# VatsalPandey0202/PointCloudRegistration

Measured on AMD Instinct MI355X. Metric: TOF/PC pairs/sec (8192 pts), higher is better.
Workload: dtype f32 xyz/features; f64 RANSAC/ICP; 1-term f16 MFMA screen (certified bound), f16x3-split MFMA screen for the rows it leaves, f64 exact re-rank; 1 GPU; C4: batch of augmented TOF/PC pairs (featNN+RANSAC+ICP+Chamfer); pairs_total=256, pairs_per_gpu=256, points=8192, feature_dim=32, streams_per_gpu=1, ransac=d=0.04 mutual n=3 edge0.9 dist0.04 (100000,0.999), icp=d=0.02 (1e-6,1e-6,30), parallelism=pair-sharded x1, inputs=resident in HBM (--full: host_resident is the PCIe-inclusive rate)

## Files before the change

pointcloudregistration_amd/csrc/featnn.hip:

```cpp
#include "featnn_v5.h"
#include "scan.h"
#include <stdlib.h>
#include <algorithm>

namespace pcr {
namespace {

__global__ __launch_bounds__(1024) void corres_build(const int32_t *nn12, const int32_t *nn21,
                                                     const int32_t *n_src, const int32_t *n_tgt,
                                                     int Nmax, int Mmax, int mutual, int ransac_n,
                                                     int *scratch, int32_t *corres,
                                                     int32_t *n_corres) {
    const int p = blockIdx.x;
    const int n = count_of(n_src, p, Nmax);
    const int m = count_of(n_tgt, p, Mmax);
    const int32_t *a12 = nn12 + (size_t)p * Nmax;
    const int32_t *a21 = nn21 + (size_t)p * Mmax;
    int *f = scratch + (size_t)p * (Nmax + 1);
    int32_t *co = corres + (size_t)p * Nmax * 2;
    for (int i = threadIdx.x; i < n; i += 1024) {
        const int j = a12[i];
        f[i] = (mutual && j >= 0 && j < m && a21[j] == i) ? 1 : 0;
    }
    __syncthreads();
// ... 147 lines not shown
static int beside(hipStream_t s, Side side, Main main) {
    static const bool off = [] {
        const char *e = getenv("PCR_FEAT_BESIDE");
        return !(e && e[0] == '1');
    }();
    hipStream_t q = s;
    hipEvent_t ef = nullptr, ej = nullptr;
    int rc = off ? PCR_OK : side_stream(&q, &ef, &ej, 2);
    if (rc != PCR_OK) return rc;
    if (q != s) {
        PCR_HIP_CHECK(hipEventRecord(ef, s));
        PCR_HIP_CHECK(hipStreamWaitEvent(q, ef, 0));
    }
    if ((rc = side(q)) != PCR_OK) return rc;
    if (q != s) PCR_HIP_CHECK(hipEventRecord(ej, q));
    prof_begin(s, kProfFeatRegroup);
    rc = main();
    prof_end(s, kProfFeatRegroup);
    if (rc != PCR_OK) return rc;
    if (q != s) PCR_HIP_CHECK(hipStreamWaitEvent(s, ej, 0));
    return PCR_OK;
}

static bool feat_one_term() {
    const char *e = getenv("PCR_FEAT_ONE");
    return !(e && e[0] == '0');
}


template <bool kIdx>
static int run_pass(const RowArgs5 &r, const RowArgs5 &fb, int S, bool one, bool use9, int slot, int slot_fb,
                    int *llist, int *lcount, hipStream_t s) {
    int rc;
    prof_begin(s, slot);
    if (use9) {
        PCR_HIP_CHECK(hipMemsetAsync(r.bcnt, 0, sizeof(int) * (size_t)r.P * (r.ntc / 2), s));
        if ((rc = launch_row9<kIdx>(r, S, s)) != PCR_OK) return rc;
        prof_end(s, slot);
        RowArgs5 rg = r;
        rg.llist = llist; rg.lcount = lcount;
        return beside(s, [&](hipStream_t q) { return launch_fallback<kIdx>(fb, S, q, slot_fb); },
                      [&] { return launch_regroup9<kIdx>(rg, S, s); });
    }
    if (one) rc = launch_row8<kIdx, true>(r, S, s);
    else if (S <= 2) rc = launch_row8<kIdx, false>(r, S, s);
    else rc = launch_row7<kIdx>(r, S, s);
    if (rc != PCR_OK) return rc;
    prof_end(s, slot);
    return one ? launch_fallback<kIdx>(fb, S, s, slot_fb) : PCR_OK;
}

static RowArgs5 fallback_args(RowArgs5 r, int *list, int *count, int fbdiag, int fsl) {
    r.rlist = r.list; r.rcount = r.count;
    r.list = list; r.count = count;
    r.fbdiag = fbdiag; r.rbmajor = 1; r.csl = fsl;
    return r;
}

static int feature_corres_v5(const float *F, const float *G, int P, int Nmax, int Mmax, int D,
                             const int32_t *n_src, const int32_t *n_tgt, int mutual, int ransac_n,
                             int32_t *nn12, int32_t *corres, int32_t *n_corres, hipStream_t s) {
    V5Buf v;
    int rc = v5_prepare(F, G, P, Nmax, Mmax, D, n_src, n_tgt, s, v);
    if (rc != PCR_OK) return rc;
    const int ntn = v.ntn, ntm = v.ntm;
    const size_t pn = (size_t)P * Nmax, pm = (size_t)P * Mmax;
    const int nst1 = ntm / 2, nst2 = ntn / 2;
    const int cap1 = std::max(64, 4 * cdiv(Nmax, nst1)), cap2 = std::max(64, 4 * cdiv(Mmax, nst2));
    const size_t pb = (size_t)P * std::max(nst1, nst2);
    const size_t pl = (size_t)P * std::max((size_t)nst1 * cap1, (size_t)nst2 * cap2);
    const size_t pr = (size_t)P * std::max(Nmax, Mmax);
    const int fsl = list_slices(P);
    const size_t pt = fsl > 1 ? (size_t)fsl * pr : 0;
    MutArgs ma;
    double *v12;
    float *e12;
    float4 *wq;
    int *nn21x, *zero, *bcnt;
    int32_t *nns;
    uint4 *blist, *rec, *part;
    WsLayout l;
    l.take(v12, pn); l.take(e12, pn);
    l.take(wq, pm);
    l.take(ma.used, pm + P); l.take(ma.pos, pm + P);
    l.take(ma.jlist, pm); l.take(nn21x, pm);
    l.take(ma.flag, pn + P);
    l.take(ma.nj, P); l.take(zero, P);
    l.take(nns, pn);
    l.take(blist, pl);
    l.take(rec, pr); l.take(part, pt);
    l.take(bcnt, pb);
    bool fresh = false;
    PCR_REQUIRE(workspace_bind(kWsFeatMutual, l, kWsSlack + 32, &fresh), PCR_ERR_NOMEM, "feature_corres: %s",
                pcr_last_error());
    const bool one = v.S <= 2 && feat_one_term();
    const bool use9 = one && feat_row9() && std::max(ntm, ntn) / 2 <= kRegroupMaxSteps;
    static thread_local const void *z_ptr = nullptr;
    static thread_local int z_cnt = 0;
    if (fresh || z_ptr != (const void *)zero || z_cnt < P) {
        PCR_HIP_CHECK(hipMemsetAsync(zero, 0, sizeof(int) * (size_t)P, s));
        z_ptr = zero;
        z_cnt = P;
    }
    ma.nn12 = nn12; ma.n_src = n_src; ma.n_tgt = n_tgt; ma.Nmax = Nmax; ma.Mmax = Mmax;
    ma.mutual = mutual; ma.ransac_n = ransac_n; ma.Kt = 16 * v.NX; ma.D = D; ma.ntm = ntm;
    ma.v12 = v12; ma.e12 = e12; ma.wq = wq; ma.fmax = v.fmax;
    ma.nns = v.S <= 2 ? nns : nn12;
    ma.F = F; ma.G = G; ma.mx = v.mx;
    ma.list21 = v.list21; ma.cnt21 = v.cnt21; ma.nn21x = nn21x;
    ma.corres = corres; ma.n_corres = n_corres;
    RowArgs5 r;
    r.Ap = v.Ap; r.Bp = v.Bp; r.rnr = v.fnr; r.cmax = v.gmax; r.n_rows = n_src; r.n_cols = n_tgt;
    r.rlist = nullptr; r.rcount = nullptr; r.P = P; r.Rmax = Nmax; r.Cmax = Mmax; r.ntr = ntn;
    r.ntc = ntm; r.nrb = 0; r.D = D; r.ctbits = 1;
    while ((1 << r.ctbits) < ntm) ++r.ctbits;
    r.nn = nn12; r.v = v12; r.e = e12;
    r.list = one ? v.fbl12 : v.list12; r.count = one ? v.fbc12 : v.cnt12;
    r.wq = nullptr;
    r.Xr = F; r.sc = v.mx; r.role = 0; r.cs = v.sp.cs;
    r.cemax = v.gemax; r.nns = nns; r.fbdiag = 0; r.rbmajor = 0;
    r.rre = v.fre; r.bcnt = bcnt; r.blist = blist; r.bcap = cap1; r.rec = rec;
    r.cct = v.gct; r.rct = v.fct; r.cbias = v.cbias;
    r.csl = 1; r.part = part; r.llist = nullptr; r.lcount = nullptr;
    auto prep_hook = [&](int at) -> int {
        if (!prep_event || prep_at != at) return PCR_OK;
        PCR_HIP_CHECK(hipEventRecord(prep_event, s));
        const int hrc = prep_fn ? prep_fn(prep_ctx) : PCR_OK;
        if (hrc == PCR_OK) prep_fn = nullptr;
        return hrc;
    };
    if ((rc = prep_hook(2)) != PCR_OK) return rc;
    rc = run_pass<true>(r, fallback_args(r, v.list12, v.cnt12, 1, fsl), v.S, one, use9, kProfFeatScreen,
                        kProfFeatScreen1b, v.list12, v.cnt12, s);
    if (rc != PCR_OK) return rc;
    if ((rc = prep_hook(1)) != PCR_OK) return rc;
    RescanArgs5 ra = rescan_args(F, G, n_src, n_tgt, Nmax, Mmax, D);
    ra.list12 = v.list12; ra.list21 = v.list21; ra.cnt12 = v.cnt12; ra.cnt21 = zero;
    ra.nn12 = nn12; ra.nn21 = nn21x;
    ra.v12 = v12; ra.e12 = e12; ra.mx = v.mx; ra.T = v.sp.T;
    hipStream_t rs = s;
    hipEvent_t ev_fork = nullptr, ev_join = nullptr;
    if (mutual && P >= 192) {
        rc = side_stream(&rs, &ev_fork, &ev_join, 1);
        if (rc != PCR_OK) return rc;
        PCR_HIP_CHECK(hipEventRecord(ev_fork, s));
        PCR_HIP_CHECK(hipStreamWaitEvent(rs, ev_fork, 0));
    }
    rc = run_rescan(ra, P, D, rs);
    if (rc != PCR_OK) return rc;
    if (rs != s) PCR_HIP_CHECK(hipEventRecord(ev_join, rs));
    if (mutual) {
        const size_t jsm = sizeof(int) * ((size_t)Mmax + 1);
        static size_t jstatic = [] {
            hipFuncAttributes fa{};
            return hipFuncGetAttributes(&fa, (const void *)featmut_jbuild<true>) == hipSuccess
                       ? fa.sharedSizeBytes : (size_t)1024;
        }();
        if (jsm + jstatic <= 64 * 1024) {
            PCR_HIP_CHECK(hipFuncSetAttribute((const void *)featmut_jbuild<true>,
                                              hipFuncAttributeMaxDynamicSharedMemorySize, 64 * 1024));
            hipLaunchKernelGGL(featmut_jbuild<true>, dim3(P), dim3(1024), jsm, s, ma);
        } else {
            hipLaunchKernelGGL(featmut_jbuild<false>, dim3(P), dim3(1024), 0, s, ma);
        }
        PCR_LAUNCH_CHECK();
        RowArgs5 r2 = r;
        r2.Ap = v.Bp; r2.Bp = v.Ap; r2.rnr = v.gnr; r2.cmax = v.fmax; r2.n_rows = n_tgt;
        r2.n_cols = n_src; r2.rlist = ma.jlist; r2.rcount = ma.nj; r2.Rmax = Mmax; r2.Cmax = Nmax;
        r2.ntr = ntm; r2.ntc = ntn;
        r2.nn = nullptr; r2.v = nullptr; r2.e = nullptr;
        r2.list = one ? v.fbl21 : nullptr; r2.count = one ? v.fbc21 : nullptr;
        r2.nns = nullptr;
        r2.wq = wq;
        r2.Xr = G; r2.sc = v.mx; r2.role = 1; r2.cs = v.sp.cs;
        r2.cemax = v.femax;
        const RowArgs5 r2b = fallback_args(r2, nullptr, nullptr, 2, fsl);
        if (use9) { r2.rre = v.gre; r2.bcap = cap2; r2.cct = v.fct; r2.rct = v.gct; }
        rc = run_pass<false>(r2, r2b, v.S, one, use9, kProfFeatScreen2, kProfFeatScreen2b, nullptr, nullptr, s);
        if (rc != PCR_OK) return rc;
        if (rs != s) PCR_HIP_CHECK(hipStreamWaitEvent(s, ev_join, 0));
        hipLaunchKernelGGL(featmut_resolve, dim3(cdiv(Nmax, 256), P), dim3(256), 0, s, ma);
        PCR_LAUNCH_CHECK();
        RescanArgs5 rb = rescan_args(F, G, n_src, n_tgt, Nmax, Mmax, D);
        rb.list12 = v.list12; rb.list21 = v.list21; rb.cnt12 = zero; rb.cnt21 = v.cnt21;
        rb.nn12 = nn12; rb.nn21 = nn21x;
        rc = run_rescan(rb, P, D, s);
        if (rc != PCR_OK) return rc;
    }
    hipLaunchKernelGGL(featmut_corres, dim3(P), dim3(1024), 0, s, ma);
    PCR_LAUNCH_CHECK();
    return PCR_OK;
}

int corres_impl(const int32_t *nn12, const int32_t *nn21, const int32_t *n_src,
                const int32_t *n_tgt, int P, int Nmax, int Mmax, int mutual, int ransac_n,
                int32_t *corres, int32_t *n_corres, hipStream_t s);

int feature_corres_impl(const float *F, const float *G, int P, int Nmax, int Mmax, int D,
                        const int32_t *n_src, const int32_t *n_tgt, int mutual, int ransac_n,
                        int32_t *nn12, int32_t *corres, int32_t *n_corres, hipStream_t s) {
    PCR_REQUIRE(D >= 1 && D <= 128, PCR_ERR_ARG, "feature_corres: D=%d unsupported (1..128)", D);
// ... 87 lines not shown
```

pointcloudregistration_amd/csrc/featnn_row.hip:

```cpp
#include "featnn_v5.h"
#include <stdlib.h>
#include <algorithm>

namespace pcr {
namespace {

__device__ unsigned long long g_featnn_fallback_rows[2];

template <int S>
__device__ __forceinline__ void row_frags(const float *x, int D, int h, int role, int cs,
                                          f16x8 (&out)[2 * S + 1]) {
    constexpr int DV = 16 * S;
    double acc = 0.0;
#pragma unroll
    for (int k = 0; k < DV; ++k)
        if (k < D) {
            const double v = (double)x[k];
            acc = acc + v * v;
        }
    _Float16 np[3];
    double wv = acc * __builtin_ldexp(1.0, -cs);
#pragma unroll
    for (int q = 0; q < 3; ++q) {
        np[q] = (_Float16)(float)wv;
// ... 210 lines not shown
                    const float m2 = __builtin_amdgcn_fmed3f(b2[t][r], ob2, -3.40282347e+38f);
                    b2[t][r] = __builtin_amdgcn_fmed3f(b1[t][r], ob1, m2);
                    b1[t][r] = __builtin_amdgcn_fmed3f(b1[t][r], ob1, -3.40282347e+38f);
                }
            }
            float mb1 = 0.f, mb2 = 0.f;
#pragma unroll
            for (int r = 0; r < 16; ++r)
                if (lr == r) { mb1 = b1[t][r]; mb2 = b2[t][r]; }
            const int k = qt * 32 + (lr & 3) + 8 * (lr >> 2) + 4 * h;
            if (lr >= 16 || k >= nr) continue;
            const int j = a.rlist[(size_t)p * a.Rmax + k];
            const double e2 = 0.5 * bound5((double)a.rnr[(size_t)p * a.ntr * 32 + j],
                                           (double)__uint_as_float(a.cmax[p]), 16 * NX, a.D);
            a.wq[(size_t)p * a.Rmax + j] = make_float4(m == 0 ? __builtin_inff() : mb1,
                                                       m == 0 ? __builtin_inff() : mb2,
                                                       (float)(e2 * (1.0 + 1e-6)), 0.0f);
        }
    }
}

constexpr int kRow8Head = 24;

__device__ __forceinline__ unsigned umin2(unsigned a, unsigned b) { return a < b ? a : b; }
__device__ __forceinline__ unsigned umax2(unsigned a, unsigned b) { return a > b ? a : b; }

#ifdef PCR_NOSCHED
#define SGB(...) ((void)0)
#else
#define SGB(...) __builtin_amdgcn_sched_group_barrier(__VA_ARGS__)
#endif
#ifndef PCR_VA
#define PCR_VA ((80 - kRow8Head + 2 * NX - 1) / (2 * NX))
#endif
#ifndef PCR_VB
#define PCR_VB ((80 - 16 + 2 * NX - 3) / (2 * NX - 2))
#endif

template <bool kIdx, bool kOne, int NX, bool kCT = false>
__device__ __forceinline__ bool row_tail(const RowArgs5 &a, int p, int row, int m, unsigned B1, unsigned B2,
                                         int mi1, float rexv, double pk, float ctr = 0.0f) {
    constexpr double kBias = kOne ? kRowBias1 : kRowBias;
    constexpr double u = 5.9604644775390625e-08;
    const double sub = kOne ? sub_term(a.D) : 0.0;
    const float mb1 = __uint_as_float(B1), mb2 = __uint_as_float(B2);
    const double qn = (double)a.rnr[(size_t)p * a.ntr * 32 + row];
    const double Gm = (double)__uint_as_float(a.cmax[p]);
    double bnd, bias, ebias = 0.0;
    if constexpr (kCT) {
        const double ex = (double)rexv + sub, E = (double)__uint_as_float(a.cemax[p]) + sub;
        const double B = (double)a.cbias[p];
        const double err = 2.0 * (16 * NX + 2) * u * ((B + Gm * Gm) + 2.0 * (qn + ex) * (Gm + E)) +
                           2.0 * (ex * Gm + (qn + ex) * E) + u * (2.0 * B + Gm * Gm) * (1.0 + 0x1p-20) + 4.0;
        bnd = 2.0 * err;
        bias = 2.0 * B - (double)ctr;
        ebias = u * (2.0 * B + qn * qn) * (1.0 + 0x1p-20);
    } else {
        bnd = (kOne ? bound1(qn, (double)rexv + sub, Gm, (double)__uint_as_float(a.cemax[p]) + sub, 16 * NX)
                    : bound5(qn, Gm, 16 * NX, a.D)) +
              4.0 * (16 * NX + 2) * u * kBias;
        bias = kBias;
    }
    if constexpr (!kIdx) {
        const double e2 = 0.5 * bnd + ebias;
        a.wq[(size_t)p * a.Rmax + row] = make_float4(m == 0 ? __builtin_inff() : mb1, m == 0 ? __builtin_inff() : mb2,
                                                     (float)(e2 * (1.0 + 1e-6)), (float)bias);
        return kOne && m != 0 && a.list &&
               !((double)mb2 - (double)mb1 > 2.0 * e2 * (1.0 + 1e-6) + 1e-6 * (double)mb1);
    }
    const size_t o = (size_t)p * a.Rmax + row;
    if (m == 0) {
        a.nn[o] = 0;
        if (a.nns) a.nns[o] = 0;
        a.v[o] = __builtin_inf();
        a.e[o] = 0.0f;
        return false;
    }
// ... 5 lines not shown
        const double dot = 2.0 * (ex * Gm + (qn + ex) * E);
        const double rest = 0.5 * bnd - dot;
        const double er = 0.5 * bnd + ebias + pk * __builtin_fabs((double)mb2);
        const double b1v = __builtin_fmax((double)mb1 - bias, 0.0);
        const double win = 2.0 * rest + 2.0 * ex * (__builtin_sqrt(b1v + 3.0 * er) + __builtin_sqrt(b1v + er)) +
                           4.0 * (qn + ex) * E;
        thr = __builtin_fmin(bnd, win * (1.0 + 1e-9));
    }
    a.nn[o] = mi1;
    if (a.nns) a.nns[o] = mi1;
    return !((double)mb2 - (double)mb1 > thr + pk * (__builtin_fabs((double)mb1) + __builtin_fabs((double)mb2)));
}

template <bool kIdx, int NX>
__device__ __forceinline__ bool one_term_fails(const RowArgs5 &a, int p, int row, unsigned B1, unsigned B2g,
                                               float rexv, float ctr) {
    constexpr double u = 5.9604644775390625e-08;
    const double sub = sub_term(a.D);
    const double mb1 = (double)__uint_as_float(B1), mb2 = (double)__uint_as_float(B2g);
    const double qn = (double)a.rnr[(size_t)p * a.ntr * 32 + row];
    const double Gm = (double)__uint_as_float(a.cmax[p]);
    const double ex = (double)rexv + sub, E = (double)__uint_as_float(a.cemax[p]) + sub;
    const double B = (double)a.cbias[p];
    const double bnd = 2.0 * (2.0 * (16 * NX + 2) * u * ((B + Gm * Gm) + 2.0 * (qn + ex) * (Gm + E)) +
                              2.0 * (ex * Gm + (qn + ex) * E) + u * (2.0 * B + Gm * Gm) * (1.0 + 0x1p-20) + 4.0);
    const double ebias = u * (2.0 * B + qn * qn) * (1.0 + 0x1p-20);
    if constexpr (!kIdx) return !(mb2 - mb1 > (bnd + 2.0 * ebias) * (1.0 + 1e-6) + 1e-6 * mb1);
    const double dot = 2.0 * (ex * Gm + (qn + ex) * E);
    const double rest = 0.5 * bnd - dot;
    const double er = 0.5 * bnd + ebias;
    const double b1v = __builtin_fmax(mb1 - (2.0 * B - (double)ctr), 0.0);
    const double win = 2.0 * rest + 2.0 * ex * (__builtin_sqrt(b1v + 3.0 * er) + __builtin_sqrt(b1v + er)) +
                       4.0 * (qn + ex) * E;
    return !(mb2 - mb1 > __builtin_fmin(bnd, win * (1.0 + 1e-9)));
}

template <int S, int G, bool kIdx, bool kOne>
__global__ __launch_bounds__(512) void featnn_row8(RowArgs5 a) {
    constexpr int W = 8, RT = 2;
    constexpr int NM = 2 * S + 1;
    constexpr int NX = kOne ? S + 1 : 3 * S + 1;
    constexpr int NB = kOne ? S + 1 : NM;
    constexpr int kB = G * NB * 64;
    constexpr double kBias = kOne ? kRowBias1 : kRowBias;
    static_assert(G % 2 == 0 && S <= 2, "column tiles in pairs; two row tiles fit up to S = 2");
    constexpr int kMerge = W * 64 * 17 * 8 / 16;
    __shared__ __attribute__((aligned(16))) f16x8 Bs[2 * kB > kMerge ? 2 * kB : kMerge];
    const int b = blockIdx.x, xcd = b & 7, slot = b >> 3;
// ... 201 lines not shown
    }
}

template <int S, bool kIdx>
__global__ __launch_bounds__(256) void featnn_slicemerge(RowArgs5 a) {
    constexpr int NX = 3 * S + 1;
    const int p = blockIdx.y, k = blockIdx.x * 256 + threadIdx.x;
    const int *rl = a.rlist + (size_t)p * a.Rmax;
    if (k >= a.rcount[p]) return;
    unsigned B1 = 0x7f800000u, B2 = 0x7f800000u, mi = 0u;
    for (int s2 = 0; s2 < a.csl; ++s2) {
        const uint4 q = a.part[((size_t)p * a.csl + s2) * a.Rmax + k];
        B2 = umin2(umin2(B2, q.y), umax2(B1, q.x));
        mi = q.x < B1 ? q.z : mi;
        B1 = umin2(B1, q.x);
    }
    const int row = rl[k];
    if (row_tail<kIdx, false, NX>(a, p, row, count_of(a.n_cols, p, a.Cmax), B1, B2, (int)mi, 0.0f,
                                  __builtin_ldexp(1.0, a.ctbits - 23)))
        a.list[(size_t)p * a.Rmax + atomicAdd(a.count + p, 1)] = row;
}


template <int S>
__device__ __forceinline__ void row_operand1(const RowArgs5 &a, int p, int row, bool valid, int h,
                                             f16x8 (&A)[S]) {
    const float sc = __uint_as_float(a.sc[p]);
    float x[16 * S];
    const float *xr = a.Xr + ((size_t)p * a.Rmax + row) * a.D;
    if (valid && a.D == 16 * S && ((uintptr_t)xr & 15) == 0) {
#pragma unroll
        for (int q = 0; q < 4 * S; ++q) {
            const float4 v = reinterpret_cast<const float4 *>(xr)[q];
            x[4 * q] = v.x * sc; x[4 * q + 1] = v.y * sc; x[4 * q + 2] = v.z * sc; x[4 * q + 3] = v.w * sc;
        }
    } else if (valid) {
#pragma unroll
        for (int q = 0; q < 16 * S; ++q) x[q] = q < a.D ? xr[q] * sc : 0.0f;
    } else {
#pragma unroll
        for (int q = 0; q < 16 * S; ++q) x[q] = 0.0f;
    }
    auto seg = [&](int k) {
        const _Float16 hi = (_Float16)x[k];
        return k < a.D ? (a.role == 0 ? (_Float16)(-2.0f * (float)hi) : hi) : (_Float16)0.0f;
    };
#pragma unroll
    for (int c = 0; c < S; ++c)
#pragma unroll
        for (int j = 0; j < 8; ++j) {
            const _Float16 v0 = seg(16 * c + j), v1 = seg(16 * c + 8 + j);
            A[c][j] = h ? v1 : v0;
        }
}

__device__ __forceinline__ f32x16 colterms(const float *tile32, int h) {
    f32x16 c;
#pragma unroll
    for (int j = 0; j < 4; ++j) {
        const float4 v = *reinterpret_cast<const float4 *>(tile32 + 8 * j + 4 * h);
        c[4 * j] = v.x; c[4 * j + 1] = v.y; c[4 * j + 2] = v.z; c[4 * j + 3] = v.w;
    }
    return c;
}

__device__ __forceinline__ unsigned fbits(float v) { return __float_as_uint(v); }

__device__ __forceinline__ unsigned group_min32(const f32x16 &x, const f32x16 &y) {
    unsigned c0 = umin2(umin2(fbits(x[0]), fbits(x[1])), fbits(x[2]));
    unsigned c1 = umin2(umin2(fbits(x[11]), fbits(x[12])), fbits(x[13]));
    unsigned c2 = umin2(umin2(fbits(y[6]), fbits(y[7])), fbits(y[8]));
#pragma unroll
    for (int r = 3; r < 11; r += 2) c0 = umin2(umin2(c0, fbits(x[r])), fbits(x[r + 1]));
    c1 = umin2(umin2(c1, fbits(x[14])), fbits(x[15]));
#pragma unroll
    for (int r = 0; r < 6; r += 2) c1 = umin2(umin2(c1, fbits(y[r])), fbits(y[r + 1]));
#pragma unroll
    for (int r = 9; r < 15; r += 2) c2 = umin2(umin2(c2, fbits(y[r])), fbits(y[r + 1]));
    c2 = umin2(c2, fbits(y[15]));
    return umin2(umin2(c0, c1), c2);
}

template <int S, int G, bool kIdx>
__global__ __launch_bounds__(512) __attribute__((amdgpu_waves_per_eu(4))) void featnn_row9(RowArgs5 a) {
    constexpr int W = 8, RT = 2;
    constexpr int NM = 2 * S + 1;
    constexpr int NB = S;
    constexpr int kT = G * NB * 64;
    constexpr int kB = kT + G * 8;
    static_assert(G % 8 == 0 && S <= 2, "column tiles in pairs; the terms in whole 1 KB DMA pieces");
// ... 151 lines not shown
    }
#pragma unroll
    for (int t = 0; t < RT; ++t) close(acc[t][1], t, pend);
    const int nst = a.ntc >> 1;
#pragma unroll
    for (int t = 0; t < RT; ++t) {
        const unsigned o1 = (unsigned)__shfl_xor((int)B1[t], 32, 64);
        const unsigned o2 = (unsigned)__shfl_xor((int)B2[t], 32, 64);
        const unsigned oi = (unsigned)__shfl_xor((int)I[t], 32, 64);
        const unsigned s2 = umin2(umax2(B1[t], o1), umin2(B2[t], o2));
        const bool mine = B1[t] < o1 || (B1[t] == o1 && h == 0);
        const unsigned w1 = mine ? B1[t] : o1;
        const unsigned wst = min(mine ? I[t] : oi, (unsigned)(nst - 1));
        const int k = (qt0 + t) * 32 + (l & 31);
        if (h == 0 && k < nr) {
            const int row = rl ? reinterpret_cast<const volatile int *>(rl)[k] : k;
            const size_t bk = (size_t)p * nst + wst;
            const bool early = one_term_fails<kIdx, S>(a, p, row, w1, s2, a.rre[(size_t)p * a.ntr * 32 + row],
                                                       a.rct[(size_t)p * a.ntr * 32 + row]);
            const int rank = early ? a.bcap : atomicAdd(a.bcnt + bk, 1);
            if (rank < a.bcap) {
                a.blist[bk * a.bcap + rank] = make_uint4((unsigned)row, w1, s2, mine ? 0u : 1u);
            } else {
                a.rec[(size_t)p * a.Rmax + row] = make_uint4(0u, 0u, 0u, 1u);
                a.list[(size_t)p * a.Rmax + atomicAdd(a.count + p, 1)] = row;
            }
        }
    }
}

template <int S, bool kIdx>
__global__ __launch_bounds__(256) __attribute__((amdgpu_waves_per_eu(4))) void featnn_regroup9(RowArgs5 a) {
    constexpr int NM = 2 * S + 1, NB = S;
    extern __shared__ int rg_lds[];
    __shared__ int wsum[4];
    const int nst = a.ntc >> 1;
    int *ts = rg_lds, *cn = rg_lds + nst + 1;
    const int nbp = gridDim.x / (8 * ((a.P + 7) >> 3));
    const int bid = blockIdx.x, xcd = bid & 7, slot = bid >> 3;
    const int p = (slot / nbp) * 8 + xcd, bx = slot % nbp;
    if (p >= a.P) return;
    const int t = threadIdx.x, wid = t >> 6, l = t & 63, h = l >> 5;
    const int *bc = a.bcnt + (size_t)p * nst;
    const int seg = (nst + 3) >> 2, s0 = min(nst, wid * seg), s1 = min(nst, s0 + seg);
    int run = 0;
    for (int c0 = s0; c0 < s1; c0 += 64) {
        const int i = c0 + l;
// ... 87 lines not shown
    const int *rl = a.rlist ? a.rlist + (size_t)p * a.Rmax : nullptr;
    const int nr = rl ? a.rcount[p] : count_of(a.n_rows, p, a.Rmax);
    const int k0 = blockIdx.x * 256 * R;
    if (k0 >= nr) return;
    const int m = count_of(a.n_cols, p, a.Cmax);
    int rows[R];
    bool put[R];
    uint4 rc[R];
#pragma unroll
    for (int i = 0; i < R; ++i) {
        const int k = k0 + i * 256 + t;
        rows[i] = k < nr ? (rl ? rl[k] : k) : -1;
        rc[i] = rows[i] >= 0 ? a.rec[(size_t)p * a.Rmax + rows[i]] : make_uint4(0u, 0u, 0u, 1u);
    }
    int mine = 0;
#pragma unroll
    for (int i = 0; i < R; ++i) {
        put[i] = false;
        if (rc[i].w == 0u)
            put[i] = row_tail<kIdx, true, S, true>(a, p, rows[i], m, rc[i].y, rc[i].z, (int)rc[i].x,
                                                   a.rre[(size_t)p * a.ntr * 32 + rows[i]], 0.0,
                                                   a.rct[(size_t)p * a.ntr * 32 + rows[i]]);
        mine += put[i] ? 1 : 0;
    }
    int x = mine;
#pragma unroll
    for (int o = 1; o < 64; o <<= 1) {
        const int y = __shfl_up(x, o, 64);
        if (l >= o) x += y;
    }
    if (l == 63) wcnt[w] = x;
    __syncthreads();
    if (t == 0) {
        const int tot = wcnt[0] + wcnt[1] + wcnt[2] + wcnt[3];
        base = tot && a.llist ? atomicAdd(a.lcount + p, tot) : 0;
    }
    __syncthreads();
    if (!a.llist) return;
    int off = base + x - mine;
    for (int ww = 0; ww < w; ++ww) off += wcnt[ww];
#pragma unroll
    for (int i = 0; i < R; ++i)
        if (put[i]) a.llist[(size_t)p * a.Rmax + off++] = rows[i];
}

}
// ... 48 lines not shown

template <bool kIdx>
int launch_regroup9(const RowArgs5 &r, int S, hipStream_t s) {
    static const int tpb = [] {
        const char *e = getenv("PCR_REGROUP_TPB");
        const int v = e ? atoi(e) : 24;
        return v >= 4 ? v : 24;
    }();
    const int nbp = cdiv(cdiv(r.Rmax, 32) + r.ntc / 2, tpb);
    const dim3 grid((unsigned)(8LL * nbp * cdiv(r.P, 8)));
    const dim3 fgrid(cdiv(r.Rmax, 1024), r.P);
    const size_t sm = sizeof(int) * (2 * (size_t)(r.ntc / 2) + 1);
    if (S == 1) {
        hipLaunchKernelGGL((featnn_regroup9<1, kIdx>), grid, dim3(256), sm, s, r);
        hipLaunchKernelGGL((featnn_finish9<1, kIdx>), fgrid, dim3(256), 0, s, r);
    } else {
        hipLaunchKernelGGL((featnn_regroup9<2, kIdx>), grid, dim3(256), sm, s, r);
        hipLaunchKernelGGL((featnn_finish9<2, kIdx>), fgrid, dim3(256), 0, s, r);
    }
    PCR_LAUNCH_CHECK();
    return PCR_OK;
}

template int launch_row7<true>(const RowArgs5 &, int, hipStream_t);
template int launch_row7<false>(const RowArgs5 &, int, hipStream_t);
template int launch_row8<true, true>(const RowArgs5 &, int, hipStream_t);
template int launch_row8<true, false>(const RowArgs5 &, int, hipStream_t);
template int launch_row8<false, true>(const RowArgs5 &, int, hipStream_t);
template int launch_row8<false, false>(const RowArgs5 &, int, hipStream_t);
template int launch_row9<true>(const RowArgs5 &, int, hipStream_t);
template int launch_row9<false>(const RowArgs5 &, int, hipStream_t);
template int launch_regroup9<true>(const RowArgs5 &, int, hipStream_t);
template int launch_regroup9<false>(const RowArgs5 &, int, hipStream_t);

}

extern "C" int pcr_featnn_fallback_rows(int64_t *rows12, int64_t *cols21, int32_t reset) {
    pcr::clear_error();
    unsigned long long v[2] = {0, 0};
    PCR_HIP_CHECK(hipDeviceSynchronize());
    PCR_HIP_CHECK(hipMemcpyFromSymbol(v, HIP_SYMBOL(pcr::g_featnn_fallback_rows), sizeof(v)));
    if (rows12) *rows12 = (int64_t)v[0];
    if (cols21) *cols21 = (int64_t)v[1];
    if (reset) {
        const unsigned long long z[2] = {0, 0};
        PCR_HIP_CHECK(hipMemcpyToSymbol(HIP_SYMBOL(pcr::g_featnn_fallback_rows), z, sizeof(z)));
// ... 4 lines not shown
```

pointcloudregistration_amd/csrc/featnn_v5.h:

```cpp
#pragma once
#include "featnn_common.h"

namespace pcr {

struct Split5 {
    int T;
    int cs;
};
inline Split5 split5_params(int D) {
    int L = 0;
    while ((1 << L) < D) ++L;
    Split5 s;
    s.T = (30 - L) / 2 < 12 ? (30 - L) / 2 : 12;
    s.cs = 2 * s.T + L - 15;
    return s;
}

namespace {

typedef _Float16 f16x8 __attribute__((ext_vector_type(8)));

__host__ __device__ constexpr int amap(int c, int S) { return c < S ? c : (c < 3 * S ? c - S : 2 * S); }
__host__ __device__ constexpr int bmap(int c, int S) { return c < 2 * S ? c : (c < 3 * S ? c - 2 * S : 2 * S); }

// ... 49 lines not shown
    int *cpi;
};

constexpr int kRow8G = 8;
#ifndef PCR_ROW9_G
#define PCR_ROW9_G 16
#endif
#ifndef PCR_ROW9_G1
#define PCR_ROW9_G1 PCR_ROW9_G
#endif
constexpr int kRow9G = PCR_ROW9_G;
constexpr int kRow9G1 = PCR_ROW9_G1;
constexpr double kRowBias = 32768.0;
constexpr double kRowBias1 = 2097152.0;

__device__ __forceinline__ double bound1(double q, double ex, double G, double E, int Kt) {
    const double u = 5.9604644775390625e-08;
    const double qg = q + G;
    const double err = 2.0 * (Kt + 2) * u * qg * qg + 2.0 * (ex * G + (q + ex) * E) +
                       1.1641532182693481e-10 * (q * q + G * G) + 4.0;
    return 2.0 * err;
}
__device__ __forceinline__ double sub_term(int D) { return 6.103515625e-05 * __builtin_sqrt((double)D); }

struct MutArgs {
    const int32_t *nn12, *n_src, *n_tgt;
    int Nmax, Mmax, mutual, ransac_n, Kt, D, ntm;
    int *used;
    int *pos;
    int *jlist, *nj;
    const double *v12;
    const float *e12;
    const float4 *wq;
    const unsigned *fmax;
    const int32_t *nns;
    const float *F, *G;
    const unsigned *mx;
    int *flag;
    int *list21, *cnt21;
    const int32_t *nn21x;
    int32_t *corres, *n_corres;
};

}

struct RescanArgs5 {
// ... 20 lines not shown
    const int *rlist, *rcount;
    int P, Rmax, Cmax, ntr, ntc, nrb, D, ctbits;
    int32_t *nn;
    double *v;
    float *e;
    int *list, *count;
    float4 *wq;
    const float *Xr;
    const unsigned *sc;
    int role, cs;
    const unsigned *cemax;
    int32_t *nns;
    int fbdiag;
    int rbmajor;
    const float *rre;
    int *bcnt, bcap;
    uint4 *blist;
    uint4 *rec;
    int *llist, *lcount;
    int csl;
    uint4 *part;
    const float *cct, *rct;
    const float *cbias;
};

struct V5Buf {
    int S, NM, NX, W, nrb, ntn, ntm, ctbits;
    Split5 sp;
    f16x8 *Ap, *Bp;
    float *fnr, *gnr;
    unsigned *gmax, *fmax, *mx;
    int *cnt12, *cnt21, *list12, *list21;
    unsigned *gemax, *femax;
    int *fbc12, *fbc21, *fbl12, *fbl21;
    float *fre, *gre;
    float *fct, *gct;
    float *cbias;
};

int v5_prepare(const float *F, const float *G, int P, int Nmax, int Mmax, int D, const int32_t *n_src,
               const int32_t *n_tgt, hipStream_t s, V5Buf &v);
int feature_match_v5(const float *F, const float *G, int P, int Nmax, int Mmax, int D, const int32_t *n_src,
                     const int32_t *n_tgt, int32_t *nn12, int32_t *nn21, hipStream_t s);
RescanArgs5 rescan_args(const float *F, const float *G, const int32_t *n_src, const int32_t *n_tgt, int Nmax,
                        int Mmax, int D);
int run_rescan(RescanArgs5 &ra, int P, int D, hipStream_t s);
constexpr int kRegroupMaxSteps = 4096;
template <bool kIdx> int launch_row7(const RowArgs5 &r, int S, hipStream_t s);
template <bool kIdx, bool kOne> int launch_row8(const RowArgs5 &r, int S, hipStream_t s);
template <bool kIdx> int launch_row9(const RowArgs5 &r, int S, hipStream_t s);
template <bool kIdx> int launch_regroup9(const RowArgs5 &r, int S, hipStream_t s);

}
```

Before: 46330 pairs/s.

## Replace f16x3 fallback with threshold candidate screen plus exact f64 re-rank

Adds a threshold pass for rows the one-term f16 screen cannot certify. It re-runs a one-term MFMA sweep that collects up to eight columns whose screened distance falls under the row's best score plus the certified error bound, then computes exact distances only for those candidates. Rows with more candidates than that are sent to the exact rescan list. This replaces the side-stream f16x3 split fallback with a cheaper bound-based filter. In exchange it adds an extra regroup launch run serially, atomics per hit, and a candidate buffer, and it can fall back to the rescan when many columns sit near the threshold.

```diff
diff --git a/pointcloudregistration_amd/csrc/featnn.hip b/pointcloudregistration_amd/csrc/featnn.hip
--- a/pointcloudregistration_amd/csrc/featnn.hip
+++ b/pointcloudregistration_amd/csrc/featnn.hip
@@ -193,6 +193,11 @@
     return PCR_OK;
 }
 
+static bool feat_thresh() {
+    const char *e = getenv("PCR_FEAT_THRESH");
+    return !(e && e[0] == '0');
+}
+
 static bool feat_one_term() {
     const char *e = getenv("PCR_FEAT_ONE");
     return !(e && e[0] == '0');
@@ -201,13 +206,25 @@
 
 template <bool kIdx>
 static int run_pass(const RowArgs5 &r, const RowArgs5 &fb, int S, bool one, bool use9, int slot, int slot_fb,
-                    int *llist, int *lcount, hipStream_t s) {
+                    int *llist, int *lcount, hipStream_t s, const RowArgs5 *th = nullptr) {
     int rc;
     prof_begin(s, slot);
     if (use9) {
         PCR_HIP_CHECK(hipMemsetAsync(r.bcnt, 0, sizeof(int) * (size_t)r.P * (r.ntc / 2), s));
         if ((rc = launch_row9<kIdx>(r, S, s)) != PCR_OK) return rc;
         prof_end(s, slot);
+        if (th) {
+            RowArgs5 rg = r;
+            rg.llist = r.list; rg.lcount = r.count; rg.thresh = 1;
+            prof_begin(s, kProfFeatRegroup);
+            rc = launch_regroup9<kIdx>(rg, S, s);
+            prof_end(s, kProfFeatRegroup);
+            if (rc != PCR_OK) return rc;
+            prof_begin(s, slot_fb);
+            rc = launch_thresh9<kIdx>(*th, S, s);
+            prof_end(s, slot_fb);
+            return rc;
+        }
         RowArgs5 rg = r;
         rg.llist = llist; rg.lcount = lcount;
         return beside(s, [&](hipStream_t q) { return launch_fallback<kIdx>(fb, S, q, slot_fb); },
@@ -243,11 +260,14 @@
     const size_t pr = (size_t)P * std::max(Nmax, Mmax);
     const int fsl = list_slices(P);
     const size_t pt = fsl > 1 ? (size_t)fsl * pr : 0;
+    const bool one = v.S <= 2 && feat_one_term();
+    const bool use9 = one && feat_row9() && std::max(ntm, ntn) / 2 <= kRegroupMaxSteps;
+    const bool thresh = use9 && feat_thresh();
     MutArgs ma;
     double *v12;
     float *e12;
     float4 *wq;
-    int *nn21x, *zero, *bcnt;
+    int *nn21x, *zero, *bcnt, *cand;
     int32_t *nns;
     uint4 *blist, *rec, *part;
     WsLayout l;
@@ -261,11 +281,10 @@
     l.take(blist, pl);
     l.take(rec, pr); l.take(part, pt);
     l.take(bcnt, pb);
+    l.take(cand, thresh ? pr * kThreshK : 0);
     bool fresh = false;
     PCR_REQUIRE(workspace_bind(kWsFeatMutual, l, kWsSlack + 32, &fresh), PCR_ERR_NOMEM, "feature_corres: %s",
                 pcr_last_error());
-    const bool one = v.S <= 2 && feat_one_term();
-    const bool use9 = one && feat_row9() && std::max(ntm, ntn) / 2 <= kRegroupMaxSteps;
     static thread_local const void *z_ptr = nullptr;
     static thread_local int z_cnt = 0;
     if (fresh || z_ptr != (const void *)zero || z_cnt < P) {
@@ -293,6 +312,7 @@
     r.rre = v.fre; r.bcnt = bcnt; r.blist = blist; r.bcap = cap1; r.rec = rec;
     r.cct = v.gct; r.rct = v.fct; r.cbias = v.cbias;
     r.csl = 1; r.part = part; r.llist = nullptr; r.lcount = nullptr;
+    r.thresh = 0; r.cand = cand; r.used = nullptr; r.Xc = G; r.fbctr = nullptr; r.dbg = 0;
     auto prep_hook = [&](int at) -> int {
         if (!prep_event || prep_at != at) return PCR_OK;
         PCR_HIP_CHECK(hipEventRecord(prep_event, s));
@@ -301,8 +321,14 @@
         return hrc;
     };
     if ((rc = prep_hook(2)) != PCR_OK) return rc;
+    auto thresh_args = [](RowArgs5 t, int *list, int *count) {
+        t.rlist = t.list; t.rcount = t.count;
+        t.llist = list; t.lcount = count;
+        return t;
+    };
+    const RowArgs5 t1 = thresh_args(r, v.list12, v.cnt12);
     rc = run_pass<true>(r, fallback_args(r, v.list12, v.cnt12, 1, fsl), v.S, one, use9, kProfFeatScreen,
-                        kProfFeatScreen1b, v.list12, v.cnt12, s);
+                        kProfFeatScreen1b, v.list12, v.cnt12, s, thresh ? &t1 : nullptr);
     if (rc != PCR_OK) return rc;
     if ((rc = prep_hook(1)) != PCR_OK) return rc;
     RescanArgs5 ra = rescan_args(F, G, n_src, n_tgt, Nmax, Mmax, D);
@@ -347,7 +373,10 @@
         r2.cemax = v.femax;
         const RowArgs5 r2b = fallback_args(r2, nullptr, nullptr, 2, fsl);
         if (use9) { r2.rre = v.gre; r2.bcap = cap2; r2.cct = v.fct; r2.rct = v.gct; }
-        rc = run_pass<false>(r2, r2b, v.S, one, use9, kProfFeatScreen2, kProfFeatScreen2b, nullptr, nullptr, s);
+        RowArgs5 t2 = thresh_args(r2, nullptr, nullptr);
+        t2.nn = nn21x; t2.used = ma.used; t2.Xc = F;
+        rc = run_pass<false>(r2, r2b, v.S, one, use9, kProfFeatScreen2, kProfFeatScreen2b, nullptr, nullptr, s,
+                             thresh ? &t2 : nullptr);
         if (rc != PCR_OK) return rc;
         if (rs != s) PCR_HIP_CHECK(hipStreamWaitEvent(s, ev_join, 0));
         hipLaunchKernelGGL(featmut_resolve, dim3(cdiv(Nmax, 256), P), dim3(256), 0, s, ma);
diff --git a/pointcloudregistration_amd/csrc/featnn_row.hip b/pointcloudregistration_amd/csrc/featnn_row.hip
--- a/pointcloudregistration_amd/csrc/featnn_row.hip
+++ b/pointcloudregistration_amd/csrc/featnn_row.hip
@@ -256,9 +256,6 @@
 
 constexpr int kRow8Head = 24;
 
-__device__ __forceinline__ unsigned umin2(unsigned a, unsigned b) { return a < b ? a : b; }
-__device__ __forceinline__ unsigned umax2(unsigned a, unsigned b) { return a > b ? a : b; }
-
 #ifdef PCR_NOSCHED
 #define SGB(...) ((void)0)
 #else
@@ -284,9 +281,7 @@
     if constexpr (kCT) {
         const double ex = (double)rexv + sub, E = (double)__uint_as_float(a.cemax[p]) + sub;
         const double B = (double)a.cbias[p];
-        const double err = 2.0 * (16 * NX + 2) * u * ((B + Gm * Gm) + 2.0 * (qn + ex) * (Gm + E)) +
-                           2.0 * (ex * Gm + (qn + ex) * E) + u * (2.0 * B + Gm * Gm) * (1.0 + 0x1p-20) + 4.0;
-        bnd = 2.0 * err;
+        bnd = bound_ct(qn, ex, Gm, E, B, 16 * NX);
         bias = 2.0 * B - (double)ctr;
         ebias = u * (2.0 * B + qn * qn) * (1.0 + 0x1p-20);
     } else {
@@ -338,8 +333,7 @@
     const double Gm = (double)__uint_as_float(a.cmax[p]);
     const double ex = (double)rexv + sub, E = (double)__uint_as_float(a.cemax[p]) + sub;
     const double B = (double)a.cbias[p];
-    const double bnd = 2.0 * (2.0 * (16 * NX + 2) * u * ((B + Gm * Gm) + 2.0 * (qn + ex) * (Gm + E)) +
-                              2.0 * (ex * Gm + (qn + ex) * E) + u * (2.0 * B + Gm * Gm) * (1.0 + 0x1p-20) + 4.0);
+    const double bnd = bound_ct(qn, ex, Gm, E, B, 16 * NX);
     const double ebias = u * (2.0 * B + qn * qn) * (1.0 + 0x1p-20);
     if constexpr (!kIdx) return !(mb2 - mb1 > (bnd + 2.0 * ebias) * (1.0 + 1e-6) + 1e-6 * mb1);
     const double dot = 2.0 * (ex * Gm + (qn + ex) * E);
@@ -587,50 +581,6 @@
 }
 
 
-template <int S>
-__device__ __forceinline__ void row_operand1(const RowArgs5 &a, int p, int row, bool valid, int h,
-                                             f16x8 (&A)[S]) {
-    const float sc = __uint_as_float(a.sc[p]);
-    float x[16 * S];
-    const float *xr = a.Xr + ((size_t)p * a.Rmax + row) * a.D;
-    if (valid && a.D == 16 * S && ((uintptr_t)xr & 15) == 0) {
-#pragma unroll
-        for (int q = 0; q < 4 * S; ++q) {
-            const float4 v = reinterpret_cast<const float4 *>(xr)[q];
-            x[4 * q] = v.x * sc; x[4 * q + 1] = v.y * sc; x[4 * q + 2] = v.z * sc; x[4 * q + 3] = v.w * sc;
-        }
-    } else if (valid) {
-#pragma unroll
-        for (int q = 0; q < 16 * S; ++q) x[q] = q < a.D ? xr[q] * sc : 0.0f;
-    } else {
-#pragma unroll
-        for (int q = 0; q < 16 * S; ++q) x[q] = 0.0f;
-    }
-    auto seg = [&](int k) {
-        const _Float16 hi = (_Float16)x[k];
-        return k < a.D ? (a.role == 0 ? (_Float16)(-2.0f * (float)hi) : hi) : (_Float16)0.0f;
-    };
-#pragma unroll
-    for (int c = 0; c < S; ++c)
-#pragma unroll
-        for (int j = 0; j < 8; ++j) {
-            const _Float16 v0 = seg(16 * c + j), v1 = seg(16 * c + 8 + j);
-            A[c][j] = h ? v1 : v0;
-        }
-}
-
-__device__ __forceinline__ f32x16 colterms(const float *tile32, int h) {
-    f32x16 c;
-#pragma unroll
-    for (int j = 0; j < 4; ++j) {
-        const float4 v = *reinterpret_cast<const float4 *>(tile32 + 8 * j + 4 * h);
-        c[4 * j] = v.x; c[4 * j + 1] = v.y; c[4 * j + 2] = v.z; c[4 * j + 3] = v.w;
-    }
-    return c;
-}
-
-__device__ __forceinline__ unsigned fbits(float v) { return __float_as_uint(v); }
-
 __device__ __forceinline__ unsigned group_min32(const f32x16 &x, const f32x16 &y) {
     unsigned c0 = umin2(umin2(fbits(x[0]), fbits(x[1])), fbits(x[2]));
     unsigned c1 = umin2(umin2(fbits(x[11]), fbits(x[12])), fbits(x[13]));
@@ -828,7 +778,7 @@
             if (rank < a.bcap) {
                 a.blist[bk * a.bcap + rank] = make_uint4((unsigned)row, w1, s2, mine ? 0u : 1u);
             } else {
-                a.rec[(size_t)p * a.Rmax + row] = make_uint4(0u, 0u, 0u, 1u);
+                a.rec[(size_t)p * a.Rmax + row] = make_uint4(0u, w1, 0xffffffffu, 1u);
                 a.list[(size_t)p * a.Rmax + atomicAdd(a.count + p, 1)] = row;
             }
         }
@@ -962,6 +912,8 @@
                                                    a.rre[(size_t)p * a.ntr * 32 + rows[i]], 0.0,
                                                    a.rct[(size_t)p * a.ntr * 32 + rows[i]]);
         mine += put[i] ? 1 : 0;
+        if (put[i] && a.thresh && a.llist)
+            a.rec[(size_t)p * a.Rmax + rows[i]] = make_uint4(0u, rc[i].y, 0xffffffffu, 1u);
     }
     int x = mine;
 #pragma unroll
@@ -1056,6 +1008,11 @@
     return PCR_OK;
 }
 
+int fallback_counter(unsigned long long **ctr) {
+    PCR_HIP_CHECK(hipGetSymbolAddress((void **)ctr, HIP_SYMBOL(g_featnn_fallback_rows)));
+    return PCR_OK;
+}
+
 template int launch_row7<true>(const RowArgs5 &, int, hipStream_t);
 template int launch_row7<false>(const RowArgs5 &, int, hipStream_t);
 template int launch_row8<true, true>(const RowArgs5 &, int, hipStream_t);
diff --git a/pointcloudregistration_amd/csrc/featnn_thresh.h b/pointcloudregistration_amd/csrc/featnn_thresh.h
--- /dev/null
+++ b/pointcloudregistration_amd/csrc/featnn_thresh.h
@@ -0,0 +1,22 @@
+#pragma once
+#include <stdint.h>
+#include <string.h>
+
+#if defined(__HIPCC__)
+#define PCR_THRESH_HD __host__ __device__
+#else
+#define PCR_THRESH_HD
+#endif
+
+namespace pcr {
+
+PCR_THRESH_HD inline uint32_t thresh_bits_up(double t) {
+    if (!(t == t)) return 0x7f800000u;
+    if (!(t > 0.0)) return 0u;
+    const float f = (float)t;
+    uint32_t b;
+    memcpy(&b, &f, sizeof(b));
+    return (double)f < t ? b + 1u : b;
+}
+
+}
diff --git a/pointcloudregistration_amd/csrc/featnn_thresh.hip b/pointcloudregistration_amd/csrc/featnn_thresh.hip
--- /dev/null
+++ b/pointcloudregistration_amd/csrc/featnn_thresh.hip
@@ -0,0 +1,244 @@
+#include "featnn_v5.h"
+#include "featnn_thresh.h"
+#include <stdlib.h>
+#include <algorithm>
+#include <cstdio>
+
+namespace pcr {
+namespace {
+
+__device__ unsigned g_thresh_stat[2][3];
+
+template <int S, bool kIdx>
+__global__ __launch_bounds__(512) void featnn_thresh9(RowArgs5 a) {
+    constexpr int NM = 2 * S + 1, NB = S, W = 8, RT = 2;
+    const int nbp = gridDim.x / (8 * ((a.P + 7) >> 3));
+    const int bid = blockIdx.x, xcd = bid & 7, slot = bid >> 3;
+    const int p = (slot / nbp) * 8 + xcd, sl = slot % nbp;
+    if (p >= a.P) return;
+    const int nr = min(a.rcount[p], a.Rmax);
+    const int m = count_of(a.n_cols, p, a.Cmax);
+    const int nst = (((m + 31) >> 5) + 1) >> 1;
+    const int nsl = min(nbp, nst);
+    if (nr <= 0 || sl >= nsl) return;
+    const int s0 = (int)((long long)nst * sl / nsl), s1 = (int)((long long)nst * (sl + 1) / nsl);
+    const int wid = threadIdx.x >> 6, l = threadIdx.x & 63, h = l >> 5;
+    const int ntl = (nr + 31) >> 5;
+    const int *rl = a.rlist + (size_t)p * a.Rmax;
+    const f16x8 *bimg = a.Bp + (size_t)p * a.ntc * NM * 64 + l;
+    const float *ctp = a.cct + (size_t)p * a.ntc * 32;
+    auto load = [&](int st, f16x8 (&Bf)[2][NB], f32x16 (&Cf)[2]) {
+#pragma unroll
+        for (int u = 0; u < 2; ++u) {
+#pragma unroll
+            for (int c = 0; c < NB; ++c) Bf[u][c] = bimg[((size_t)(2 * st + u) * NM + c) * 64];
+            Cf[u] = colterms(ctp + (size_t)(2 * st + u) * 32, h);
+        }
+    };
+    for (int t0 = wid * RT; t0 < ntl; t0 += W * RT) {
+        size_t o[RT];
+        unsigned B1[RT], thr[RT], am[RT];
+        bool live[RT];
+        int nh[RT];
+        f16x8 A[RT][NB];
+#pragma unroll
+        for (int t = 0; t < RT; ++t) {
+            const int k = (t0 + t) * 32 + (l & 31);
+            const bool valid = k < nr;
+            const int row = valid ? rl[k] : 0;
+            o[t] = (size_t)p * a.Rmax + row;
+            B1[t] = valid ? a.rec[o[t]].y : 0x7f800000u;
+            thr[t] = 0u;
+            live[t] = false;
+            if (valid && B1[t] < 0x7f800000u) {
+                const double bnd = row_bound_ct(a, p, row, a.rre[(size_t)p * a.ntr * 32 + row], 16 * S);
+                thr[t] = thresh_bits_up((double)__uint_as_float(B1[t]) + bnd * (1.0 + 0x1p-20));
+                live[t] = thr[t] < 0x7f800000u;
+            }
+            row_operand1<S>(a, p, row, valid, h, A[t]);
+            am[t] = 0xffffffffu;
+            nh[t] = 0;
+        }
+        f16x8 Bf[2][NB];
+        f32x16 Cf[2];
+        load(s0, Bf, Cf);
+        for (int st = s0; st < s1; ++st) {
+            f16x8 Bn[2][NB];
+            f32x16 Cn[2];
+            load(st + 1 < s1 ? st + 1 : st, Bn, Cn);
+            f32x16 acc[RT][2];
+#pragma unroll
+            for (int c = 0; c < NB; ++c)
+#pragma unroll
+                for (int u = 0; u < 2; ++u)
+#pragma unroll
+                    for (int t = 0; t < RT; ++t)
+                        acc[t][u] = __builtin_amdgcn_mfma_f32_32x32x16_f16(Bf[u][c], A[t][c],
+                                                                           c == 0 ? Cf[u] : acc[t][u], 0, 0, 0);
+#pragma unroll
+            for (int t = 0; t < RT; ++t)
+#pragma unroll
+                for (int u = 0; u < 2; ++u) {
+                    unsigned long long any = 0ull;
+#pragma unroll
+                    for (int r = 0; r < 16; ++r) any |= __ballot(fbits(acc[t][u][r]) <= thr[t]);
+                    if (any == 0ull) continue;
+#pragma unroll
+                    for (int r = 0; r < 16; ++r) {
+                        const unsigned v = fbits(acc[t][u][r]);
+                        const int col = 32 * (2 * st + u) + 8 * (r >> 2) + 4 * h + (r & 3);
+                        if (v <= thr[t] && live[t] && col < m) {
+                            if (kIdx && v == B1[t]) am[t] = umin2(am[t], (unsigned)col);
+                            if (nh[t] <= kThreshK) {
+                                const unsigned pos = atomicAdd(reinterpret_cast<unsigned *>(a.rec + o[t]), 1u);
+                                if (pos < (unsigned)kThreshK) a.cand[o[t] * kThreshK + pos] = col;
+                            }
+                            ++nh[t];
+                        }
+                    }
+                }
+#pragma unroll
+            for (int u = 0; u < 2; ++u) {
+#pragma unroll
+                for (int c = 0; c < NB; ++c) Bf[u][c] = Bn[u][c];
+                Cf[u] = Cn[u];
+            }
+        }
+#pragma unroll
+        for (int t = 0; t < RT; ++t)
+            if (kIdx && am[t] != 0xffffffffu) atomicMin(reinterpret_cast<unsigned *>(a.rec + o[t]) + 2, am[t]);
+    }
+}
+
+template <int DV, bool kIdx>
+__global__ __launch_bounds__(256) void featnn_exact_cand(RowArgs5 a) {
+    const int p = blockIdx.y;
+    const int nr = min(a.rcount[p], a.Rmax);
+    if (nr <= 0) return;
+    if (blockIdx.x == 0 && threadIdx.x == 0) atomicAdd(a.fbctr + (kIdx ? 0 : 1), (unsigned long long)nr);
+    const int m = count_of(a.n_cols, p, a.Cmax);
+    const int *rl = a.rlist + (size_t)p * a.Rmax;
+    const int c = threadIdx.x & 7, rr = threadIdx.x >> 3, D = a.D;
+    const float4 open = make_float4(__builtin_inff(), __builtin_inff(), __builtin_inff(), 0.0f);
+    for (int k0 = blockIdx.x * 32; k0 < nr; k0 += gridDim.x * 32) {
+        const bool act = k0 + rr < nr;
+        const int row = act ? rl[k0 + rr] : 0;
+        const size_t o = (size_t)p * a.Rmax + row;
+        const uint4 rc = act ? a.rec[o] : make_uint4(0u, 0x7f800000u, 0u, 1u);
+        const int cnt = (int)min(rc.x, (unsigned)kThreshK + 1u);
+        double best = __builtin_inf();
+        int bj = 0x7fffffff;
+        if (act && m > 0 && c < cnt && cnt <= kThreshK && rc.y < 0x7f800000u) {
+            const int j = a.cand[o * kThreshK + c];
+            const float *q = a.Xr + o * D, *y = a.Xc + ((size_t)p * a.Cmax + j) * D;
+            float qf[DV], yf[DV];
+            if (D == DV && (((uintptr_t)q | (uintptr_t)y) & 15) == 0) {
+#pragma unroll
+                for (int k = 0; k < DV; k += 4) {
+                    const float4 u = *reinterpret_cast<const float4 *>(q + k), w = *reinterpret_cast<const float4 *>(y + k);
+                    qf[k] = u.x; qf[k + 1] = u.y; qf[k + 2] = u.z; qf[k + 3] = u.w;
+                    yf[k] = w.x; yf[k + 1] = w.y; yf[k + 2] = w.z; yf[k + 3] = w.w;
+                }
+            } else {
+#pragma unroll
+                for (int k = 0; k < DV; ++k) {
+                    qf[k] = k < D ? q[k] : 0.0f;
+                    yf[k] = k < D ? y[k] : 0.0f;
+                }
+            }
+            double acc = 0.0;
+#pragma unroll
+            for (int k = 0; k < DV; ++k) {
+                const double df = (double)qf[k] - (double)yf[k];
+                acc = acc + df * df;
+            }
+            if (acc < best) { best = acc; bj = j; }
+        }
+#pragma unroll
+        for (int x = 1; x < 8; x <<= 1) {
+            const double ob = __shfl_xor(best, x, 64);
+            const int oj = __shfl_xor(bj, x, 64);
+            if (ob < best || (ob == best && oj < bj)) { best = ob; bj = oj; }
+        }
+        if (c != 0 || !act) continue;
+        if (m == 0) {
+            if constexpr (kIdx) {
+                a.nn[o] = 0;
+                a.nns[o] = 0;
+                a.v[o] = __builtin_inf();
+                a.e[o] = 0.0f;
+            } else {
+                a.wq[o] = open;
+            }
+            continue;
+        }
+        if constexpr (kIdx) a.nns[o] = rc.z < (unsigned)m ? (int)rc.z : 0;
+        const bool over = bj == 0x7fffffff;
+        if (a.dbg) {
+            atomicAdd(&g_thresh_stat[kIdx ? 0 : 1][0], 1u);
+            atomicMax(&g_thresh_stat[kIdx ? 0 : 1][1], rc.x);
+            if (over) atomicAdd(&g_thresh_stat[kIdx ? 0 : 1][2], 1u);
+        }
+        if constexpr (kIdx) {
+            if (over) {
+                a.llist[(size_t)p * a.Rmax + atomicAdd(a.lcount + p, 1)] = row;
+            } else {
+                const double sc = (double)__uint_as_float(a.sc[p]);
+                a.nn[o] = bj;
+                a.v[o] = best * sc * sc;
+                a.e[o] = 0.0f;
+            }
+        } else {
+            a.wq[o] = open;
+            if (!over) {
+                a.nn[o] = bj;
+                a.used[(size_t)p * (a.Rmax + 1) + row] = 2;
+            }
+        }
+    }
+}
+
+}
+
+static int thresh_blocks_per_pair(int P) {
+    static const int forced = [] {
+        const char *e = getenv("PCR_THRESH_SLICES");
+        return e ? atoi(e) : 0;
+    }();
+    if (forced >= 1 && forced <= 128) return forced;
+    return std::max(4, std::min(32, 1024 / std::max(P, 1)));
+}
+
+template <bool kIdx>
+int launch_thresh9(const RowArgs5 &r0, int S, hipStream_t s) {
+    RowArgs5 r = r0;
+    static const bool dbg = getenv("PCR_THRESH_DEBUG") != nullptr;
+    r.dbg = dbg ? 1 : 0;
+    int rc = fallback_counter(&r.fbctr);
+    if (rc != PCR_OK) return rc;
+    const int nbp = thresh_blocks_per_pair(r.P);
+    const dim3 grid((unsigned)(8LL * nbp * cdiv(r.P, 8)));
+    if (S == 1) hipLaunchKernelGGL((featnn_thresh9<1, kIdx>), grid, dim3(512), 0, s, r);
+    else hipLaunchKernelGGL((featnn_thresh9<2, kIdx>), grid, dim3(512), 0, s, r);
+    PCR_LAUNCH_CHECK();
+    const dim3 eg(std::min(8, cdiv(r.Rmax, 32)), r.P);
+    if (S == 1) hipLaunchKernelGGL((featnn_exact_cand<16, kIdx>), eg, dim3(256), 0, s, r);
+    else hipLaunchKernelGGL((featnn_exact_cand<32, kIdx>), eg, dim3(256), 0, s, r);
+    PCR_LAUNCH_CHECK();
+    if (dbg) {
+        unsigned st[2][3];
+        PCR_HIP_CHECK(hipStreamSynchronize(s));
+        PCR_HIP_CHECK(hipMemcpyFromSymbol(st, HIP_SYMBOL(g_thresh_stat), sizeof(st)));
+        const int d = kIdx ? 0 : 1;
+        fprintf(stderr, "thresh pass %d: listed %u, max candidates %u, to the exact rescan %u\n", d + 1, st[d][0],
+                st[d][1], st[d][2]);
+        const unsigned z[3] = {0, 0, 0};
+        PCR_HIP_CHECK(hipMemcpyToSymbol(HIP_SYMBOL(g_thresh_stat), z, sizeof(z), sizeof(z) * d));
+    }
+    return PCR_OK;
+}
+
+template int launch_thresh9<true>(const RowArgs5 &, int, hipStream_t);
+template int launch_thresh9<false>(const RowArgs5 &, int, hipStream_t);
+
+}
diff --git a/pointcloudregistration_amd/csrc/featnn_v5.h b/pointcloudregistration_amd/csrc/featnn_v5.h
--- a/pointcloudregistration_amd/csrc/featnn_v5.h
+++ b/pointcloudregistration_amd/csrc/featnn_v5.h
@@ -95,6 +95,29 @@
     return 2.0 * err;
 }
 __device__ __forceinline__ double sub_term(int D) { return 6.103515625e-05 * __builtin_sqrt((double)D); }
+
+__device__ __forceinline__ double bound_ct(double q, double ex, double G, double E, double B, int Kt) {
+    const double u = 5.9604644775390625e-08;
+    const double err = 2.0 * (Kt + 2) * u * ((B + G * G) + 2.0 * (q + ex) * (G + E)) +
+                       2.0 * (ex * G + (q + ex) * E) + u * (2.0 * B + G * G) * (1.0 + 0x1p-20) + 4.0;
+    return 2.0 * err;
+}
+
+__device__ __forceinline__ unsigned umin2(unsigned a, unsigned b) { return a < b ? a : b; }
+__device__ __forceinline__ unsigned umax2(unsigned a, unsigned b) { return a > b ? a : b; }
+__device__ __forceinline__ unsigned fbits(float v) { return __float_as_uint(v); }
+
+__device__ __forceinline__ f32x16 colterms(const float *tile32, int h) {
+    f32x16 c;
+#pragma unroll
+    for (int j = 0; j < 4; ++j) {
+        const float4 v = *reinterpret_cast<const float4 *>(tile32 + 8 * j + 4 * h);
+        c[4 * j] = v.x; c[4 * j + 1] = v.y; c[4 * j + 2] = v.z; c[4 * j + 3] = v.w;
+    }
+    return c;
+}
+
+constexpr int kThreshK = 8;
 
 struct MutArgs {
     const int32_t *nn12, *n_src, *n_tgt;
@@ -161,7 +184,55 @@
     uint4 *part;
     const float *cct, *rct;
     const float *cbias;
-};
+    int thresh;
+    int *cand, *used;
+    const float *Xc;
+    unsigned long long *fbctr;
+    int dbg;
+};
+
+namespace {
+
+template <int S>
+__device__ __forceinline__ void row_operand1(const RowArgs5 &a, int p, int row, bool valid, int h,
+                                             f16x8 (&A)[S]) {
+    const float sc = __uint_as_float(a.sc[p]);
+    float x[16 * S];
+    const float *xr = a.Xr + ((size_t)p * a.Rmax + row) * a.D;
+    if (valid && a.D == 16 * S && ((uintptr_t)xr & 15) == 0) {
+#pragma unroll
+        for (int q = 0; q < 4 * S; ++q) {
+            const float4 v = reinterpret_cast<const float4 *>(xr)[q];
+            x[4 * q] = v.x * sc; x[4 * q + 1] = v.y * sc; x[4 * q + 2] = v.z * sc; x[4 * q + 3] = v.w * sc;
+        }
+    } else if (valid) {
+#pragma unroll
+        for (int q = 0; q < 16 * S; ++q) x[q] = q < a.D ? xr[q] * sc : 0.0f;
+    } else {
+#pragma unroll
+        for (int q = 0; q < 16 * S; ++q) x[q] = 0.0f;
+    }
+    auto seg = [&](int k) {
+        const _Float16 hi = (_Float16)x[k];
+        return k < a.D ? (a.role == 0 ? (_Float16)(-2.0f * (float)hi) : hi) : (_Float16)0.0f;
+    };
+#pragma unroll
+    for (int c = 0; c < S; ++c)
+#pragma unroll
+        for (int j = 0; j < 8; ++j) {
+            const _Float16 v0 = seg(16 * c + j), v1 = seg(16 * c + 8 + j);
+            A[c][j] = h ? v1 : v0;
+        }
+}
+
+__device__ __forceinline__ double row_bound_ct(const RowArgs5 &a, int p, int row, float rexv, int Kt) {
+    const double sub = sub_term(a.D);
+    return bound_ct((double)a.rnr[(size_t)p * a.ntr * 32 + row], (double)rexv + sub,
+                    (double)__uint_as_float(a.cmax[p]), (double)__uint_as_float(a.cemax[p]) + sub,
+                    (double)a.cbias[p], Kt);
+}
+
+}
 
 struct V5Buf {
     int S, NM, NX, W, nrb, ntn, ntm, ctbits;
@@ -189,5 +260,7 @@
 template <bool kIdx, bool kOne> int launch_row8(const RowArgs5 &r, int S, hipStream_t s);
 template <bool kIdx> int launch_row9(const RowArgs5 &r, int S, hipStream_t s);
 template <bool kIdx> int launch_regroup9(const RowArgs5 &r, int S, hipStream_t s);
-
-}
+int fallback_counter(unsigned long long **ctr);
+template <bool kIdx> int launch_thresh9(const RowArgs5 &r, int S, hipStream_t s);
+
+}
```

Result: faster. 48810 pairs/s, median of 6 (+5.4%).
